# LuoGuiwen/MSM_blst

Measured on AMD Instinct MI355X. Metric: G1 MSM point-scalar pairs/sec at n=2^20, 1/2/4/8 MI355X; bit-exact vs CPU, higher is better.
Workload: dtype u32 (exact Fp381 integer arithmetic, 14x28-bit limbs)

## Files before the change

### msm_blst_amd/csrc/ches.hip

```cpp
#include <hipcub/hipcub.hpp>

#include <algorithm>
#include <cstdlib>
#include <cstring>

#include "ches_kernels.hpp"
#include "coop.hpp"
#include "engine.hpp"
#include "hoststage.hpp"
#include "pair_kernels.hpp"

#ifndef MSM_GROUP
#error "define MSM_GROUP (1 or 2)"
#endif

namespace msm {

#if MSM_GROUP == 1
static const ChesParams kChesTable[] = {
    {8, 0, 12, 22, 7, 6, 857, 10, 26},         {9, 0, 13, 20, 231, 6, 1725, 11, 24},
    {10, 0, 13, 20, 231, 6, 1725, 12, 22},     {11, 0, 14, 19, 7, 6, 3417, 13, 20},
    {12, 0, 14, 19, 7, 6, 3417, 13, 20},       {13, 0, 16, 16, 29677, 6, 18343, 15, 17},
    {14, 0, 16, 16, 29677, 6, 18343, 15, 17},  {15, 0, 16, 16, 29677, 6, 18343, 16, 16},
    {16, 0, 19, 14, 231, 6, 109244, 17, 15},   {16, 1, 18, 15, 7, 6, 54618, 17, 15},
// ... 1020 lines not shown
  const size_t fs_bytes = fg_max * n * (size_t)p_.h * 16 + 1;
  const int nfr = phase ? (int)std::max<size_t>(kFrontsMax, std::min<size_t>(kFrontPhase, ((size_t)4 << 30) / fs_bytes))
                        : nl >= 2 ? kFrontsMax : kFronts;
  const int nred = nl >= 2 ? 4 : 2;
  if ((int)fs_.size() < nfr) fs_.resize(nfr);
  for (int t = 0; t < nred; ++t) red.ensure_group(t, (int)group_max);
  const size_t sslot = n * stride;
  bool unsized = false;
  for (int f = 0; f < nfr; ++f) unsized |= fs_[f].sorted.bytes < n * (size_t)p_.h * fg_max * 4;
  static const size_t nsg_env = [] {
    const char *e = getenv("MSM_H2D_SLOTS");
    return (size_t)(e ? std::max(2, std::min(256, atoi(e))) : 0);
  }();
  const size_t slot_groups =
      std::max<size_t>(nsg_env ? nsg_env : std::max<size_t>(4, std::min<size_t>(32, ((size_t)2 << 30) / (fg_max * sslot))),
                       (size_t)nfr - 1);
  const size_t nsg = std::max<size_t>(std::min(slot_groups, nfg), (size_t)nfr - 1);
  if (scalars_on_host) scal_.ensure(slot_groups * fg_max * sslot + 16);
  if (unsized) scal_.ensure(fg_max * sslot + 16);
  for (int f = 0; f < nfr; ++f)
    if (fs_[f].sorted.bytes < n * (size_t)p_.h * fg_max * 4) {
      MSM_HIP_CHECK(hipMemsetAsync(scal_.p, 0, fg_max * sslot, s));
      digits_sort(s, scal_.as<uint8_t>(), stride, sslot, (int)fg_max, f);
      MSM_HIP_CHECK(hipStreamSynchronize(s));
    }
  const bool prof = profile_;
  profile_ = false;
  if (prof)
    while (acc_ev_.size() < std::max<size_t>(2 * count, 2 * 64)) {
      hipEvent_t e;
      MSM_HIP_CHECK(hipEventCreate(&e));
      acc_ev_.push_back(e);
    }
  while (bev_.size() < std::max<size_t>(3 * count + 2 * nfg + ngroups + 1, 3 * 64 + 3 * 64 + 1)) {
    hipEvent_t e;
    MSM_HIP_CHECK(hipEventCreateWithFlags(&e, hipEventDisableTiming));
    bev_.push_back(e);
  }
  hipEvent_t *eva = bev_.data() + 1, *evh = eva + count, *evf = evh + count, *evc = evf + nfg, *evt = evc + nfg;
  std::vector<size_t> prof_k;
  MSM_HIP_CHECK(hipEventRecord(bev_[0], s));
  MSM_HIP_CHECK(hipStreamWaitEvent(fstream_, bev_[0], 0));
  if (scalars_on_host) MSM_HIP_CHECK(hipEventSynchronize(bev_[0]));
  for (int t = 0; t < kBSets; ++t) MSM_HIP_CHECK(hipStreamWaitEvent(tails_[t], bev_[0], 0));
  auto slots = [&](size_t g) { return scal_.as<uint8_t>() + (g % nsg) * fg_max * sslot; };
  static const bool zc_env = [] {
    const char *e = getenv("MSM_ZERO_COPY_SCALARS");
    return e && atoi(e) != 0;
  }();
  bool zero_copy = false;
  if (scalars_on_host && zc_env) {
    hipPointerAttribute_t a;
    zero_copy = hipPointerGetAttributes(&a, scalars) == hipSuccess && a.type == hipMemoryTypeHost;
    if (!zero_copy) (void)hipGetLastError();
  }
  auto copy_group = [&](size_t g) {
    if (!scalars_on_host || zero_copy || g >= nfg) return;
    if (g >= nsg) MSM_HIP_CHECK(hipStreamWaitEvent(cstream_, evf[g - nsg], 0));
    for (size_t k = fgb[g]; k < fgb[g + 1]; ++k)
      MSM_HIP_CHECK(hipMemcpyAsync(slots(g) + (k - fgb[g]) * sslot, job_scalars(k), sslot, hipMemcpyHostToDevice,
                                   cstream_));
    MSM_HIP_CHECK(hipEventRecord(evc[g], cstream_));
  };
  static const bool front_after_l0 = [] {
    const char *e = getenv("MSM_FRONT_AFTER_L0");
    return e && atoi(e) != 0;
  }();
  static const size_t pace_env = [] {
    const char *e = getenv("MSM_COPY_PACE");
    return (size_t)(e ? std::max(0, std::min(32, atoi(e))) : 8);
  }();
  const size_t pace = scalars_on_host && !zero_copy && pace_env >= 3 ? pace_env : 0;
  size_t acc_enq = 0;
  auto front_group = [&](size_t g) {
    if (g >= nfg) return;
    const bool copied = scalars_on_host && !zero_copy;
    if (pace && g >= pace && g < nsg) {
      if (acc_enq) MSM_HIP_CHECK(hipEventSynchronize(eva[std::min(fgb[g] - pace, acc_enq - 1)]));
      copy_group(g);
    }
    if (copied) MSM_HIP_CHECK(hipStreamWaitEvent(fstream_, evc[g], 0));
    if (g >= (size_t)nfr) {
      const size_t last = fgb[g - nfr + 1] - 1;
      MSM_HIP_CHECK(hipStreamWaitEvent(fstream_, eva[last], 0));
      if (front_after_l0 && nl < 2) MSM_HIP_CHECK(hipStreamWaitEvent(fstream_, evh[last], 0));
      for (size_t d = 1; d < (size_t)nl && last >= d && last - d >= fgb[g - nfr]; ++d)
        MSM_HIP_CHECK(hipStreamWaitEvent(fstream_, eva[last - d], 0));
    }
    const uint8_t *src = copied ? slots(g) : job_scalars(fgb[g]);
    digits_sort(fstream_, src, stride, copied ? sslot : jstride, (int)(fgb[g + 1] - fgb[g]), (int)(g % nfr),
                fine_bt);
    MSM_HIP_CHECK(hipEventRecord(evf[g], fstream_));
  };
  for (size_t g = 0; g < (pace ? std::min(nsg, pace) : nsg); ++g) copy_group(g);
  static const int l0_env = [] {
    const char *e = getenv("MSM_ACC_AFTER_L0");
    return e ? (atoi(e) != 0 ? 1 : 0) : -1;
  }();
  const bool l0_first = l0_env < 0 ? G == 1 : l0_env == 1;
  size_t fronts_issued = 0;
  auto issue_fronts = [&](size_t upto) {
    for (; fronts_issued <= upto && fronts_issued < nfg; ++fronts_issued) front_group(fronts_issued);
  };
  const size_t nphase = phase ? std::min(nfg, (size_t)nfr) : 1;
  issue_fronts(nphase - 1);
  if (acc_groups) {
    hipStream_t lane[2] = {s, tails_[0]}, ts = tails_[1];
    for (size_t g = 0; g < nfg; ++g) {
      copy_group(g + nsg);
      const size_t k0 = fgb[g], k1 = fgb[g + 1];
      const int gb = (int)(g & 1);
      hipStream_t L = lane[gb];
      MSM_HIP_CHECK(hipStreamWaitEvent(L, evf[g], 0));
      if (g == 0 && nphase > 1) MSM_HIP_CHECK(hipStreamWaitEvent(L, evf[nphase - 1], 0));
      if (prof) MSM_HIP_CHECK(hipEventRecord(acc_ev_[2 * k0], L));
      accumulate_sets(L, (int)(g % nfr), (int)(k1 - k0), gb, job_table(k0));
      if (prof) {
        MSM_HIP_CHECK(hipEventRecord(acc_ev_[2 * k0 + 1], L));
        prof_k.push_back(k0);
      }
      for (size_t k = k0; k < k1; ++k) MSM_HIP_CHECK(hipEventRecord(eva[k], L));
      acc_enq = k1;
      for (size_t a = k0; a < k1;) {
        const size_t q = grp(a), b = std::min(k1, gfirst[q + 1]);
        if (q >= (size_t)nred) MSM_HIP_CHECK(hipStreamWaitEvent(L, evt[q - nred], 0));
        red.launch_head_slots(L, gbuckets_[gb].as<uint8_t>() + (a - k0) * NB * sizeof(Xyzz<typename FieldOf<G>::F>), NB,
                              (int)(q % nred), (int)gslot(a), (int)(b - a));
        a = b;
      }
      for (size_t k = k0; k < k1; ++k) MSM_HIP_CHECK(hipEventRecord(evh[k], L));
      for (size_t k = k0; k < k1; ++k) {
        if (!gend(k)) continue;
        const size_t q = grp(k), first = gfirst[q];
        MSM_HIP_CHECK(hipStreamWaitEvent(ts, evh[k], 0));
        if (k0 >= 1 && k0 - 1 >= first) MSM_HIP_CHECK(hipStreamWaitEvent(ts, evh[k0 - 1], 0));
        group_tail(ts, (int)(q % nred), first, k - first + 1, k + 1 == count);
        MSM_HIP_CHECK(hipEventRecord(evt[q], ts));
      }
      issue_fronts(g + nfr - 1);
    }
  }
  if (nl >= 2 && !acc_groups) {
    hipStream_t lane[3] = {s, tails_[0], tails_[1]}, ts = nl == 3 ? fstream_ : tails_[1];
    for (size_t g = 0; g < nfg; ++g) {
      copy_group(g + nsg);
      for (size_t k = fgb[g]; k < fgb[g + 1]; ++k) {
        hipStream_t L = lane[k % nl];
        const size_t q = grp(k);
        const int bset = (int)(k % nl), slot = (int)gslot(k), gset = (int)(q % nred);
        MSM_HIP_CHECK(hipStreamWaitEvent(L, evf[g], 0));
        if (q >= (size_t)nred && slot < nl)
          MSM_HIP_CHECK(hipStreamWaitEvent(L, evt[q - nred], 0));
        if (prof) MSM_HIP_CHECK(hipEventRecord(acc_ev_[2 * k], L));
        accumulate(L, (int)(g % nfr), (int)(k - fgb[g]), bset, job_table(k));
        if (prof) {
          MSM_HIP_CHECK(hipEventRecord(acc_ev_[2 * k + 1], L));
          prof_k.push_back(k);
        }
        MSM_HIP_CHECK(hipEventRecord(eva[k], L));
        acc_enq = k + 1;
        red.launch_head_slot(L, buckets_[bset].p, gset, slot);
        MSM_HIP_CHECK(hipEventRecord(evh[k], L));
        if (gend(k)) {
          for (int d = 0; d < nl && d <= slot; ++d) MSM_HIP_CHECK(hipStreamWaitEvent(ts, evh[k - d], 0));
          group_tail(ts, gset, k - slot, slot + 1, k + 1 == count);
          MSM_HIP_CHECK(hipEventRecord(evt[q], ts));
        }
      }
      issue_fronts(g + nfr - 1);
    }
  }
  static const int fuse_env = [] {
    const char *e = getenv("MSM_L0_FUSE");
    return e ? std::max(0, std::min(2, atoi(e))) : 0;
  }();
  const int fuse = nl < 2 ? fuse_env : 0;
  auto l0_group_tail = [&](size_t p) {
    const size_t pq = grp(p), pslot = gslot(p);
    if (!gend(p)) return;
    hipStream_t ts = tails_[pq % 2];
    MSM_HIP_CHECK(hipStreamWaitEvent(ts, evh[p], 0));
    group_tail(ts, (int)(pq % 2), p - pslot, pslot + 1, p + 1 == count);
    MSM_HIP_CHECK(hipEventRecord(evt[pq], ts));
  };
  auto l0_set_free = [&](size_t p) {
    const size_t pq = grp(p);
    if (gslot(p) == 0 && pq >= 2) MSM_HIP_CHECK(hipStreamWaitEvent(s, evt[pq - 2], 0));
  };
  for (size_t g = 0; g < (nl >= 2 || !fuse ? 0 : nfg); ++g) {
    copy_group(g + nsg);
    MSM_HIP_CHECK(hipStreamWaitEvent(s, evf[g], 0));
    for (size_t k = fgb[g]; k < fgb[g + 1]; ++k) {
      const int bset = (int)(k % kBSets);
      if (k >= 1) l0_set_free(k - 1);
      if (prof) MSM_HIP_CHECK(hipEventRecord(acc_ev_[2 * k], s));
      if (k >= 1)
        accumulate_l0(s, (int)(g % nfr), (int)(k - fgb[g]), bset, job_table(k), (int)((k - 1) % kBSets),
                      (int)(grp(k - 1) % 2), (int)gslot(k - 1), fuse == 2);
      else
        accumulate(s, (int)(g % nfr), (int)(k - fgb[g]), bset, job_table(k));
      if (prof) {
        MSM_HIP_CHECK(hipEventRecord(acc_ev_[2 * k + 1], s));
        prof_k.push_back(k);
      }
      MSM_HIP_CHECK(hipEventRecord(eva[k], s));
      acc_enq = k + 1;
      if (k >= 1) {
        MSM_HIP_CHECK(hipEventRecord(evh[k - 1], s));
        l0_group_tail(k - 1);
      }
    }
    issue_fronts(g + nfr - 1);
  }
  if (fuse && nl < 2) {
    const size_t p = count - 1;
    l0_set_free(p);
    red.launch_head_slot(s, buckets_[p % kBSets].p, (int)(grp(p) % 2), (int)gslot(p));
    MSM_HIP_CHECK(hipEventRecord(evh[p], s));
    l0_group_tail(p);
  }
  for (size_t g = 0; g < (nl >= 2 || fuse ? 0 : nfg); ++g) {
    copy_group(g + nsg);
    MSM_HIP_CHECK(hipStreamWaitEvent(s, evf[g], 0));
    for (size_t k = fgb[g]; k < fgb[g + 1]; ++k) {
      const int bset = (int)(k % kBSets), slot = (int)gslot(k), gset = (int)(grp(k) % 2);
      hipStream_t ts = tails_[gset];
      if (k >= (size_t)kBSets) MSM_HIP_CHECK(hipStreamWaitEvent(s, evh[k - kBSets], 0));
      if (l0_first && k >= 1) MSM_HIP_CHECK(hipStreamWaitEvent(s, evh[k - 1], 0));
      if (prof) MSM_HIP_CHECK(hipEventRecord(acc_ev_[2 * k], s));
      accumulate(s, (int)(g % nfr), (int)(k - fgb[g]), bset, job_table(k));
      if (prof) {
        MSM_HIP_CHECK(hipEventRecord(acc_ev_[2 * k + 1], s));
        prof_k.push_back(k);
      }
      MSM_HIP_CHECK(hipEventRecord(eva[k], s));
      acc_enq = k + 1;
      MSM_HIP_CHECK(hipStreamWaitEvent(ts, eva[k], 0));
      red.launch_head_slot(ts, buckets_[bset].p, gset, slot);
      MSM_HIP_CHECK(hipEventRecord(evh[k], ts));
      if (gend(k)) {
        group_tail(ts, gset, k - slot, slot + 1, k + 1 == count);
      }
    }
    issue_fronts(g + nfr - 1);
  }
  MSM_HIP_CHECK(hipEventRecord(ev_tail_[0], fstream_));
  MSM_HIP_CHECK(hipStreamWaitEvent(s, ev_tail_[0], 0));
  for (int t = 0; t < kBSets; ++t) {
    MSM_HIP_CHECK(hipEventRecord(ev_tail_[t], tails_[t]));
    MSM_HIP_CHECK(hipStreamWaitEvent(s, ev_tail_[t], 0));
  }
  for (int t = 0; t < kBSets; ++t) MSM_HIP_CHECK(hipStreamSynchronize(tails_[t]));
  MSM_HIP_CHECK(hipStreamSynchronize(fstream_));
  const size_t last_first = gfirst[ngroups - 1];
  auto combine_k = [&](size_t k) {
    outs[k] = bit_tail && k >= last_first ? red.combine_bits((const uint8_t *)host_bits_ + (k - last_first) * bb)
                                          : red.combine((const uint8_t *)host_out_ + k * ob)[0];
  };
  if (dev_out) {
  } else if (count >= 4) {
    WorkerPool::get().parallel_for(count, combine_k);
// ... 22 lines not shown
```

### msm_blst_amd/csrc/ches_kernels.hpp

```cpp
#pragma once
#include "bucket_sort.hpp"
#include "kernels.hpp"

namespace msm {

constexpr uint32_t CH_IDX_MASK = 0x00ffffffu;

__device__ constexpr uint64_t PM2[6] = {0xb9feffffffffaaa9ull, 0x1eabfffeb153ffffull, 0x6730d2a0f6b0f624ull,
                                        0x64774b84f38512bfull, 0x4b1ba7b6434bacd7ull, 0x1a0111ea397fe69aull};
__device__ __forceinline__ void fp_inv(Fp &r, const Fp &a) {
  Fp a1 = a, a2, a3, acc;
  fp_norm(a1);
  fp_sqr(a2, a1);
  fp_mul(a3, a2, a1);
  fp_one(acc);
  for (int k = 190; k >= 0; --k) {
    if (k != 190) {
      fp_sqr(acc, acc);
      fp_sqr(acc, acc);
    }
    const uint32_t w = (uint32_t)(PM2[k >> 5] >> ((k & 31) * 2)) & 3u;
    if (w) {
      const uint32_t m1 = 0u - (uint32_t)(w == 1), m2 = 0u - (uint32_t)(w == 2), m3 = 0u - (uint32_t)(w == 3);
      Fp t;
// ... 381 lines not shown
    return (int32_t)((uint32_t)((((uint64_t)hi << 32) | lo) >> sh) & qmask);
  };
  int32_t carry = 0;
  for (int j = 0; j < h - 1; ++j) carry = digit(j) + carry > qh ? 1 : 0;
  uint32_t neg = 0;
  if (digit(h - 1) + carry > qh) {
    r_minus(s);
    neg = 1u;
  }
  carry = 0;
  for (int j = 0; j < h; ++j) {
    int32_t d = digit(j) + carry;
    carry = 0;
    if (j < h - 1 && d > qh) {
      d -= q;
      carry = 1;
    }
    const size_t k = (size_t)j * n + i;
    if (d == 0) {
      keys[k] = KEY_NONE;
      continue;
    }
    uint32_t sign = (d < 0 ? 1u : 0u) ^ neg;
    uint32_t b = (uint32_t)(d < 0 ? -d : d) - 1u;
    if (j == h - 1 && b < small) {
      uint32_t c = (uint32_t)(i % copies);
      if (c) b = nb0 + (c - 1) * small + b;
    }
    keys[k] = b;
    vals[k] = (uint32_t)(i * (size_t)h + j) | (sign << 31);
  }
}

#ifndef MSM_SEGSUM_PREFETCH
#define MSM_SEGSUM_PREFETCH 0
#endif
#ifndef MSM_SEGSUM_CHAIN
#define MSM_SEGSUM_CHAIN 0
#endif
template <int G>
struct SegsumForm {
  typedef MulSplit T;
};
#if MSM_SEGSUM_CHAIN
template <>
struct SegsumForm<1> {
  typedef MulChain T;
};
#endif
template <int G>
__device__ __forceinline__ void segsum_one(const Xyzz<typename FieldOf<G>::F> *__restrict__ src,
                                           const uint32_t *__restrict__ idx, const uint32_t *__restrict__ starts,
                                           Xyzz<typename FieldOf<G>::F> *__restrict__ dst, size_t t) {
  typedef typename FieldOf<G>::F F;
  uint32_t lo = starts[t], hi = starts[t + 1];
  Xyzz<F> acc;
  if (lo == hi) {
    xyzz_set_inf(acc);
  } else {
    acc = ld16(&src[idx ? idx[lo] : lo]);
#if MSM_SEGSUM_PREFETCH
    Xyzz<F> nxt;
    if (lo + 1 < hi) nxt = ld16(&src[idx ? idx[lo + 1] : lo + 1]);
    for (uint32_t k = lo + 1; k < hi; ++k) {
      Xyzz<F> a = nxt;
      if (k + 1 < hi) nxt = ld16(&src[idx ? idx[k + 1] : k + 1]);
      xyzz_add<F, AddRegrouped<F>::value, typename SegsumForm<G>::T>(acc, a);
    }
#else
    for (uint32_t k = lo + 1; k < hi; ++k) {
      Xyzz<F> a = ld16(&src[idx ? idx[k] : k]);
      xyzz_add<F, AddRegrouped<F>::value, typename SegsumForm<G>::T>(acc, a);
    }
#endif
  }
  st16(&dst[t], acc);
}
template <int G>
static __global__ void __launch_bounds__(256)
    k_segsum(const Xyzz<typename FieldOf<G>::F> *__restrict__ src, const uint32_t *__restrict__ idx,
             const uint32_t *__restrict__ starts, Xyzz<typename FieldOf<G>::F> *__restrict__ dst, size_t nout,
             size_t src_stride, size_t dst_stride) {
  size_t t = (size_t)blockIdx.x * blockDim.x + threadIdx.x;
  if (t >= nout) return;
  segsum_one<G>(src + blockIdx.y * src_stride, idx, starts, dst + blockIdx.y * dst_stride, t);
}

template <class PT>
static __global__ void __launch_bounds__(256, MSM_ACC_WAVES)
    k_accumulate_l0(const AccSched S, const PT *__restrict__ pts, Xyzz<Fp> *__restrict__ buckets, size_t nbuckets,
                    const Xyzz<Fp> *__restrict__ l0src, const uint32_t *__restrict__ l0idx,
                    const uint32_t *__restrict__ l0starts, Xyzz<Fp> *__restrict__ l0dst, size_t l0out,
                    uint32_t l0blocks, int l0_last) {
  const uint32_t nacc = gridDim.x - l0blocks;
  const bool l0 = l0_last ? blockIdx.x >= nacc : blockIdx.x < l0blocks;
  const uint32_t b = l0 ? (l0_last ? blockIdx.x - nacc : blockIdx.x) : (l0_last ? blockIdx.x : blockIdx.x - l0blocks);
  const size_t t = (size_t)b * blockDim.x + threadIdx.x;
  if (l0) {
    if (t < l0out) segsum_one<1>(l0src, l0idx, l0starts, l0dst, t);
  } else if (t < nbuckets) {
    accumulate_bucket<1>(S, pts, buckets, t);
  }
}

template <int G>
static __global__ void __launch_bounds__(64)
    k_suffix_step(const Xyzz<typename FieldOf<G>::F> *__restrict__ in, Xyzz<typename FieldOf<G>::F> *__restrict__ out,
                  int S, int d, int W) {
  typedef typename FieldOf<G>::F F;
  size_t t = (size_t)blockIdx.x * blockDim.x + threadIdx.x;
  if (t >= (size_t)W * S) return;
  int k = (int)(t % (size_t)S);
  Xyzz<F> a = ld16(&in[t]);
  if (k + d < S) {
    Xyzz<F> b = ld16(&in[t + d]);
    xyzz_add(a, b);
  }
  st16(&out[t], a);
}
template <int G>
static __global__ void __launch_bounds__(64)
    k_pair_step(const Xyzz<typename FieldOf<G>::F> *__restrict__ in, Xyzz<typename FieldOf<G>::F> *__restrict__ out,
                size_t nout) {
  typedef typename FieldOf<G>::F F;
  size_t t = (size_t)blockIdx.x * blockDim.x + threadIdx.x;
  if (t >= nout) return;
  Xyzz<F> a = ld16(&in[2 * t]);
  Xyzz<F> b = ld16(&in[2 * t + 1]);
  xyzz_add(a, b);
  st16(&out[t], a);
}


template <int G>
__global__ void __launch_bounds__(256) k_import_xyzz(const uint64_t *__restrict__ in, Xyzz<typename FieldOf<G>::F> *__restrict__ out,
// ... 35 lines not shown
```

### include/msm_mi355x.h

```cpp
#ifndef MSM_MI355X_H
#define MSM_MI355X_H

#include <stddef.h>
#include <stdint.h>

#ifdef __cplusplus
extern "C" {
#endif

typedef uint8_t byte;
typedef uint64_t limb_t;
typedef struct { byte b[256 / 8]; } blst_scalar;
typedef struct { limb_t l[384 / 8 / sizeof(limb_t)]; } blst_fp;
typedef struct { blst_fp fp[2]; } blst_fp2;
typedef struct { blst_fp x, y, z; } blst_p1;
typedef struct { blst_fp x, y; } blst_p1_affine;
typedef struct { blst_fp2 x, y, z; } blst_p2;
typedef struct { blst_fp2 x, y; } blst_p2_affine;
typedef struct { blst_fp x, y, zzz, zz; } blst_p1xyzz;
typedef struct { blst_fp2 x, y, zzz, zz; } blst_p2xyzz;
typedef struct { int m; int b; int alpha; } digit_decomposition;

size_t blst_p1s_mult_pippenger_scratch_sizeof(size_t npoints);
void blst_p1s_mult_pippenger(blst_p1 *ret, const blst_p1_affine *const points[], size_t npoints,
// ... 68 lines not shown
                                   const int scalars[], const unsigned char booth_signs[], blst_p2xyzz buckets[],
                                   size_t q_exponent);

void blst_p1s_add(blst_p1 *ret, const blst_p1_affine *const points[], size_t npoints);
void blst_p2s_add(blst_p2 *ret, const blst_p2_affine *const points[], size_t npoints);

size_t blst_p1s_mult_wbits_precompute_sizeof(size_t wbits, size_t npoints);
void blst_p1s_mult_wbits_precompute(blst_p1_affine table[], size_t wbits, const blst_p1_affine *const points[],
                                    size_t npoints);
size_t blst_p1s_mult_wbits_scratch_sizeof(size_t npoints);
void blst_p1s_mult_wbits(blst_p1 *ret, const blst_p1_affine table[], size_t wbits, size_t npoints,
                         const byte *const scalars[], size_t nbits, limb_t *scratch);
size_t blst_p2s_mult_wbits_precompute_sizeof(size_t wbits, size_t npoints);
void blst_p2s_mult_wbits_precompute(blst_p2_affine table[], size_t wbits, const blst_p2_affine *const points[],
                                    size_t npoints);
size_t blst_p2s_mult_wbits_scratch_sizeof(size_t npoints);
void blst_p2s_mult_wbits(blst_p2 *ret, const blst_p2_affine table[], size_t wbits, size_t npoints,
                         const byte *const scalars[], size_t nbits, limb_t *scratch);

enum {
  MSM_OK = 0,
  MSM_E_ARG = -1,
  MSM_E_HIP = -2,
  MSM_E_NODEV = -3,
  MSM_E_STATE = -4
};
typedef struct msm_ctx msm_ctx;
const char *msm_last_error(void);
int msm_set_abort_on_error(int on);
int msm_error_pending(void);
int msm_device_count(void);
int msm_valu_probe(int device, double out[4]);
int msm_fp_form_ops(int device, int form, const uint32_t *in, size_t lanes, uint32_t *out);
void msm_release_engine_cache(void);
void msm_engine_cache_stats(size_t out[3]);
size_t msm_set_engine_cache_limit(size_t bytes);
int msm_register_host_table(int group, const void *rows_affine, size_t nrows);
int msm_unregister_host_table(const void *rows_affine);
int msm_ctx_create(msm_ctx **ctx, int group, int device, int window_bits);
int msm_ctx_set_points(msm_ctx *ctx, const void *points_affine, size_t npoints, int points_on_device,
                       void *hip_stream);
int msm_ctx_mult(msm_ctx *ctx, void *ret, const byte *scalars, size_t stride, size_t nbits, int scalars_on_device,
                 void *hip_stream);
int msm_ctx_mult_batch(msm_ctx *ctx, void *rets, const byte *scalars, size_t stride, size_t set_stride,
                       size_t nbits, size_t count, int scalars_on_device, void *hip_stream);
int msm_ctx_set_profiling(msm_ctx *ctx, int on);
int msm_ctx_phase_times(const msm_ctx *ctx, float out[6]);
void msm_ctx_destroy(msm_ctx *ctx);

typedef struct msm_ches_ctx msm_ches_ctx;
int msm_ches_params(int n_exp, int beta, int out[9]);
int msm_ches_ctx_create(msm_ches_ctx **ctx, int group, int device, int n_exp, int beta);
int msm_ches_ctx_create_params(msm_ches_ctx **ctx, int group, int device, const int params[9]);
int msm_ches_ctx_create_multi(msm_ches_ctx **ctx, int group, const int *devices, int ndev, int n_exp, int beta);
int msm_ches_ctx_shards(const msm_ches_ctx *ctx);
int msm_ches_ctx_rccl_exchange(const msm_ches_ctx *ctx);
int msm_ches_ctx_build_table(msm_ches_ctx *ctx, const void *points_affine, size_t npoints, int on_device,
                             void *hip_stream);
int msm_ches_ctx_set_table(msm_ches_ctx *ctx, const void *table_affine, size_t npoints, int on_device,
                           void *hip_stream);
int msm_ches_ctx_get_table(msm_ches_ctx *ctx, void *out_affine, size_t first, size_t count);
int msm_ches_ctx_mult(msm_ches_ctx *ctx, void *ret, const byte *scalars, size_t stride, int scalars_on_device,
                      void *hip_stream);
int msm_ches_ctx_mult_batch(msm_ches_ctx *ctx, void *rets, const byte *scalars, size_t stride, size_t set_stride,
                            size_t count, int scalars_on_device, void *hip_stream);
int msm_ches_ctx_save_table(msm_ches_ctx *ctx, const char *path);
// ... 135 lines not shown
```

### msm_blst_amd/csrc/abi.cpp

```cpp
#include <hip/hip_runtime.h>
#include <stdio.h>
#include <stdlib.h>
#include <string.h>

#include <algorithm>
#include <atomic>
#include <map>
#include <memory>
#include <mutex>
#include <string>

#include "../../include/msm_mi355x.h"
#include "decode.hpp"
#include "encode.hpp"
#include "engine.hpp"
#include "hash_to_curve.hpp"
#include "multi.hpp"
#include "pairing.hpp"
#include "point_segments.hpp"
#include "points_mult.hpp"
#include "pool.hpp"
#include "ptr_walk.hpp"
#include "sig_verify.hpp"
#include "table_registry.hpp"
// ... 1246 lines not shown
int msm_unregister_host_table(const void *rows) {
  if (!rows) return fail(MSM_E_ARG, "null rows");
  return TableRegistry::get().remove(rows) ? MSM_OK : fail(MSM_E_ARG, "table not registered");
}

int msm_device_count(void) {
  int n = 0;
  if (hipGetDeviceCount(&n) != hipSuccess) return 0;
  return n;
}

int msm_valu_probe(int device, double out[4]) {
  if (!out) return fail(MSM_E_ARG, "null out");
  if (msm_device_count() <= device || device < 0) return fail(MSM_E_NODEV, "no such HIP device");
  try {
    valu_probe(device, out);
    return MSM_OK;
  } catch (const std::exception &e) {
    return fail(MSM_E_HIP, e.what());
  }
}

int msm_fp_form_ops(int device, int form, const uint32_t *in, size_t lanes, uint32_t *out) {
  if (!in || !out || !lanes || (form != 0 && form != 1)) return fail(MSM_E_ARG, "bad in / out / lanes / form");
  if (msm_device_count() <= device || device < 0) return fail(MSM_E_NODEV, "no such HIP device");
  try {
    form_ops(device, form, in, lanes, out);
    return MSM_OK;
  } catch (const std::exception &e) {
    return fail(MSM_E_HIP, e.what());
  }
}

int msm_ctx_create(msm_ctx **ctx, int group, int device, int window_bits) {
  if (!ctx || (group != 1 && group != 2)) return fail(MSM_E_ARG, "bad ctx/group");
  if (msm_device_count() <= device || device < 0) return fail(MSM_E_NODEV, "no such HIP device");
  try {
    auto c = std::make_unique<msm_ctx>();
    c->group = group;
    c->device = device;
    int wb = window_bits > 0 ? window_bits : 16;
    if (group == 1) c->g1 = std::make_unique<Pippenger<1>>(device, wb);
    else c->g2 = std::make_unique<Pippenger<2>>(device, wb);
    *ctx = c.release();
    return MSM_OK;
  } catch (const std::exception &e) {
    return fail(MSM_E_HIP, e.what());
  }
}

int msm_ctx_set_points(msm_ctx *ctx, const void *points, size_t n, int on_device, void *stream) {
  if (!ctx || (!points && n)) return fail(MSM_E_ARG, "bad args");
  try {
    if (ctx->group == 1) ctx->g1->set_points(points, n, on_device != 0, (hipStream_t)stream);
    else ctx->g2->set_points(points, n, on_device != 0, (hipStream_t)stream);
    return MSM_OK;
  } catch (const std::exception &e) {
    return fail(MSM_E_HIP, e.what());
  }
}

int msm_ctx_set_points_encoded(msm_ctx *ctx, const void *src, size_t n, int encoding, int flags, int src_on_device,
                               size_t *first_bad, void *stream) {
  if (!ctx || (!src && n)) return fail(MSM_E_ARG, "bad args");
  if (n == 0) return msm_ctx_set_points(ctx, nullptr, 0, 1, stream);
  std::vector<uint8_t> st;
// ... 640 lines not shown
```

### msm_blst_amd/csrc/ec.hpp

```cpp
#pragma once
#include "fp.hpp"

namespace msm {

template <class F>
struct Aff {
  F x, y;
};
template <class F>
struct Xyzz {
  F x, y, zzz, zz;
};

template <class F>
MSM_FN bool xyzz_is_inf(const Xyzz<F> &a) {
  return f_is_zero_exact(a.zz);
}
template <class F>
MSM_FN void xyzz_set_inf(Xyzz<F> &a) {
  f_zero(a.x);
  f_zero(a.y);
  f_zero(a.zzz);
  f_zero(a.zz);
}
// ... 5 lines not shown
    f_nred(r.y);
  } else {
    r.y = p.y;
  }
  f_one(r.zzz);
  f_one(r.zz);
}

template <class F, class CF = MulSplit>
MSM_FN void xyzz_dbl(Xyzz<F> &r, const Xyzz<F> &a) {
  if (xyzz_is_inf(a)) {
    r = a;
    return;
  }
  F U, V, W, S, M, t, X3;
  f_add(U, a.y, a.y);
  f_sqr(V, U, CF{});
  f_mul(W, V, U, CF{});
  f_mul(S, a.x, V, CF{});
  f_mul(r.zz, V, a.zz, CF{});
  f_mul(r.zzz, W, a.zzz, CF{});
  f_sqr(M, a.x, CF{});
  f_mul3(M, M);
  f_sqr(X3, M, CF{});
  F z;
  f_zero(z);
  f_sub_2x(X3, X3, z, S);
  f_norm(X3);
  f_sub16(t, S, X3);
  f_mul_sub(r.y, t, M, W, a.y, CF{});
  r.x = X3;
}

template <class F, class CF = MulSplit>
MSM_FN void xyzz_madd(Xyzz<F> &acc, const Aff<F> &p, bool neg, bool acc_affine = false) {
  if (xyzz_is_inf(acc)) {
    xyzz_from_aff(acc, p, neg);
    return;
  }
  F y2, P, R, PP, PPP, t;
  if (neg) {
    f_neg4(y2, p.y);
  } else {
    y2 = p.y;
  }
  if (acc_affine) {
    P = p.x;
    if (neg) f_nred(y2);
    R = y2;
  } else {
    f_mul_bs(P, p.x, acc.zz, CF{});
    f_mul_bs(R, y2, acc.zzz, CF{});
  }
  f_sub16(P, P, acc.x);
  f_sub4(R, R, acc.y);
  f_sqr(PP, P, CF{});
  if (__builtin_expect(f_is_zero_S(PP), 0)) {
    F RR;
    f_sqr(RR, R, CF{});
    if (f_is_zero_S(RR)) {
      Xyzz<F> b = acc;
      xyzz_dbl<F, CF>(acc, b);
    } else {
      xyzz_set_inf(acc);
    }
    return;
  }
  if (!__builtin_constant_p(acc_affine)) f_pin(PP);
  if (acc_affine) {
    acc.zz = PP;
  } else {
    f_mul_bs(acc.zz, acc.zz, PP, CF{});
  }
  f_mul_bs(PPP, P, PP, CF{});
  f_mul_bs(acc.x, acc.x, PP, CF{});
  if (acc_affine) {
    acc.zzz = PPP;
  } else {
    f_mul_bs(acc.zzz, acc.zzz, PPP, CF{});
  }
  F X3;
  f_sqr(X3, R, CF{});
  f_sub_2x(X3, X3, PPP, acc.x);
  f_norm(X3);
  f_sub16(t, acc.x, X3);
  f_mul_sub(acc.y, t, R, acc.y, PPP, CF{});
  acc.x = X3;
}

template <class F, class CF = MulSplit>
MSM_FN void xyzz_add_u1s1(Xyzz<F> &acc, const Xyzz<F> &b) {
  F P, R, PP, PPP, t;
  f_mul_bs(acc.x, acc.x, b.zz, CF{});
  f_mul_bs(acc.y, acc.y, b.zzz, CF{});
  f_mul_bs(P, b.x, acc.zz, CF{});
  f_sub4(P, P, acc.x);
  f_mul_bs(R, b.y, acc.zzz, CF{});
  f_sub4(R, R, acc.y);
  f_mul_bs(acc.zz, acc.zz, b.zz, CF{});
  f_mul_bs(acc.zzz, acc.zzz, b.zzz, CF{});
  f_sqr(PP, P, CF{});
  if (__builtin_expect(f_is_zero_S(PP), 0)) {
    F RR;
    f_sqr(RR, R, CF{});
    if (f_is_zero_S(RR)) {
      Xyzz<F> a = acc;
      xyzz_dbl<F, CF>(acc, a);
    } else {
      xyzz_set_inf(acc);
    }
    return;
  }
  f_mul_bs(acc.zz, acc.zz, PP, CF{});
  f_mul_bs(PPP, P, PP, CF{});
  f_mul_bs(acc.x, acc.x, PP, CF{});
  f_mul_bs(acc.zzz, acc.zzz, PPP, CF{});
  F X3;
  f_sqr(X3, R, CF{});
  f_sub_2x(X3, X3, PPP, acc.x);
  f_norm(X3);
// ... 59 lines not shown
```

### msm_blst_amd/csrc/engine.hpp

```cpp
#pragma once
#include <hip/hip_runtime.h>
#include <stdint.h>

#include <cstdlib>
#include <memory>
#include <stdexcept>
#include <string>
#include <vector>

#include "acc_sched.hpp"
#include "host_fp.hpp"

#define MSM_HIP_CHECK(x)                                                                           \
  do {                                                                                            \
    hipError_t e_ = (x);                                                                          \
    if (e_ != hipSuccess)                                                                         \
      throw std::runtime_error(std::string("HIP error ") + hipGetErrorString(e_) + " at " + #x); \
  } while (0)

namespace msm {

class HostStager;

inline unsigned nblk(size_t n, unsigned b) { return (unsigned)((n + b - 1) / b); }
// ... 370 lines not shown
class Wbits {
 public:
  typedef typename HostField<G>::F HF;
  Wbits(int device, int wbits);
  void precompute(const void *points_blst, size_t n, bool on_device, hipStream_t s);
  void set_table(const void *table_blst, size_t n, bool on_device, hipStream_t s);
  void get_table(void *out_blst, size_t first, size_t count, hipStream_t s);
  void run(hipStream_t s, const uint8_t *d_scalars, size_t stride, int nbits, hfp::Jac<HF> *out);
  void upload_scalars(const void *host, size_t bytes, hipStream_t s);
  size_t npoints() const { return n_; }
  size_t table_rows() const { return n_ << (wbits_ - 1); }
  int wbits() const { return wbits_; }
  int device() const { return dev_; }
  size_t device_bytes() const { return table_.bytes + parts_[0].bytes + parts_[1].bytes + fin_.bytes + scal_.bytes; }

 private:
  int dev_, wbits_;
  size_t n_ = 0;
  DevBuf table_, parts_[2], fin_, scal_;
};

template <int G>
void entry_msm(void *ret_jac, const void *pts_blst, size_t npts, const uint32_t *keys, const uint32_t *vals,
               size_t ne, size_t nb, const uint32_t *weights, void *buckets_out);
typedef void (*EntryFill)(void *ctx, size_t t0, size_t t1, uint32_t *keys, uint32_t *vals);
template <int G>
void entry_msm_ptrs(void *ret, const void *const *points, size_t ne, EntryFill fill, void *fill_ctx, size_t nb,
                    const uint32_t *weights, void *buckets_out);
template <int G>
void weighted_bucket_sum(void *ret_jac, const void *buckets_blst, size_t nb, const uint32_t *weights);

void valu_probe(int device, double out[4]);
void form_ops(int device, int form, const uint32_t *in, size_t lanes, uint32_t *out);
template <int G>
void test_field(int op, const uint64_t *a, const uint64_t *b, uint64_t *out, size_t n);
template <int G>
void test_xyzz(const uint64_t *pts, size_t npts, const uint32_t *ops, int len, size_t nseq, uint64_t *out);

struct DeviceGuard {
  int prev = -1;
  explicit DeviceGuard(int dev) {
    MSM_HIP_CHECK(hipGetDevice(&prev));
    if (prev != dev) MSM_HIP_CHECK(hipSetDevice(dev));
  }
  ~DeviceGuard() {
    int cur = -1;
    if (hipGetDevice(&cur) == hipSuccess && cur != prev && prev >= 0) (void)hipSetDevice(prev);
  }
};

}
```

### msm_blst_amd/csrc/probe.hip

```cpp
#include <hip/hip_runtime.h>

#include <algorithm>
#include <cstring>

#include "kernels.hpp"
#include "engine.hpp"

namespace msm {
namespace {

__global__ void __launch_bounds__(256) k_probe_mad(uint64_t *out, uint32_t seed, int iters) {
  const uint32_t t = threadIdx.x + blockIdx.x * blockDim.x;
  uint64_t acc[16];
  const uint32_t a = t | 1, b = seed | 3;
#pragma unroll
  for (int k = 0; k < 16; ++k) acc[k] = t + k;
  for (int it = 0; it < iters; ++it) {
#pragma unroll
    for (int k = 0; k < 16; ++k)
      asm volatile("v_mad_u64_u32 %0, vcc, %1, %2, %0" : "+v"(acc[k]) : "v"(a), "v"(b) : "vcc");
  }
  uint64_t s = 0;
#pragma unroll
  for (int k = 0; k < 16; ++k) s += acc[k];
// ... 30 lines not shown
  for (int it = 0; it < 2 * iters; ++it) {
    const Aff<Fp> p = pts[it & 3];
    xyzz_madd(acc, p, (it & 2) != 0);
  }
  uint32_t s = 0;
#pragma unroll
  for (int i = 0; i < NL; ++i) s ^= acc.x.v[i] ^ acc.y.v[i] ^ acc.zzz.v[i] ^ acc.zz.v[i];
  out[t] = s;
}

template <class CF>
__global__ void __launch_bounds__(256) k_form_ops(const Fp *__restrict__ in, Fp *__restrict__ out, size_t lanes) {
  const size_t t = (size_t)blockIdx.x * blockDim.x + threadIdx.x;
  if (t >= lanes) return;
  const Fp *a = in + t * 8;
  Fp *o = out + t * 11;
  Fp r;
  fp_mul(r, a[0], a[1], CF{});
  o[0] = r;
  fp_sqr(r, a[0], CF{});
  o[1] = r;
  fp_mul2(r, a[0], a[1], a[2], a[3], CF{});
  o[2] = r;
  Xyzz<Fp> q = {a[0], a[1], a[2], a[3]};
  const Aff<Fp> p = {a[4], a[5]};
  xyzz_madd<Fp, CF>(q, p, (t & 1) != 0);
  o[3] = q.x, o[4] = q.y, o[5] = q.zzz, o[6] = q.zz;
  q = {a[0], a[1], a[2], a[3]};
  const Xyzz<Fp> b = {a[4], a[5], a[6], a[7]};
  xyzz_add<Fp, true, CF>(q, b);
  o[7] = q.x, o[8] = q.y, o[9] = q.zzz, o[10] = q.zz;
}

template <class L>
float best_ms(L launch) {
  hipEvent_t e0, e1;
  MSM_HIP_CHECK(hipEventCreate(&e0));
  MSM_HIP_CHECK(hipEventCreate(&e1));
  launch();
  MSM_HIP_CHECK(hipGetLastError());
  MSM_HIP_CHECK(hipDeviceSynchronize());
  float best = 1e30f;
  for (int r = 0; r < 3; ++r) {
    MSM_HIP_CHECK(hipEventRecord(e0, 0));
    launch();
    MSM_HIP_CHECK(hipEventRecord(e1, 0));
    MSM_HIP_CHECK(hipEventSynchronize(e1));
    float ms = 0;
    MSM_HIP_CHECK(hipEventElapsedTime(&ms, e0, e1));
    best = std::min(best, ms);
  }
  (void)hipEventDestroy(e0);
  (void)hipEventDestroy(e1);
  return best;
}

}

void valu_probe(int device, double out[4]) {
  {
    DeviceGuard g(device);
    int cus = 0;
    MSM_HIP_CHECK(hipDeviceGetAttribute(&cus, hipDeviceAttributeMultiprocessorCount, device));
    DevBuf obuf, pbuf;
    obuf.ensure((size_t)cus * 8 * 256 * 8);
    Aff<Fp> h[4];
// ... 24 lines not shown
      total += 4 * ms;
      fpm = std::max(fpm, (double)blocks * 256 * iters * 2 / (ms * 1e-3));
    }
    for (int bpc : {3, 6}) {
      const int blocks = cus * bpc, iters = 64;
      const float ms = best_ms([&] {
        hipLaunchKernelGGL(k_probe_madd, dim3(blocks), dim3(256), 0, 0, obuf.as<uint32_t>(), pbuf.as<Aff<Fp>>(),
                           iters);
      });
      total += 4 * ms;
      madd = std::max(madd, (double)blocks * 256 * iters * 2 / (ms * 1e-3));
    }
    out[0] = mad;
    out[1] = fpm;
    out[2] = madd;
    out[3] = total;
  }
}

void form_ops(int device, int form, const uint32_t *in, size_t lanes, uint32_t *out) {
  DeviceGuard g(device);
  DevBuf ibuf, obuf;
  ibuf.ensure(lanes * 8 * sizeof(Fp));
  obuf.ensure(lanes * 11 * sizeof(Fp));
  MSM_HIP_CHECK(hipMemcpy(ibuf.p, in, lanes * 8 * sizeof(Fp), hipMemcpyHostToDevice));
  const dim3 grid((unsigned)((lanes + 255) / 256));
  if (form) hipLaunchKernelGGL(k_form_ops<MulChain>, grid, dim3(256), 0, 0, ibuf.as<Fp>(), obuf.as<Fp>(), lanes);
  else hipLaunchKernelGGL(k_form_ops<MulSplit>, grid, dim3(256), 0, 0, ibuf.as<Fp>(), obuf.as<Fp>(), lanes);
  MSM_HIP_CHECK(hipGetLastError());
  MSM_HIP_CHECK(hipDeviceSynchronize());
  MSM_HIP_CHECK(hipMemcpy(out, obuf.p, lanes * 11 * sizeof(Fp), hipMemcpyDeviceToHost));
}

}
```

Baseline: 483.9 million.

## Add kernel-based H2D scalar staging and pace host copies on accumulate start

Adds an opt-in path, MSM_H2D_STAGE, that copies host scalars into the device slot buffers with a vectorized non-temporal-load GPU kernel reading mapped host memory, in place of per-job hipMemcpyAsync. That path can run on the copy or front stream and is gated on stream events with a configurable lead. The default pacing of host scalar copies also changes. When fewer than two accumulation lanes are used, the host now waits on new per-job accumulate-start events with a shorter pace, not on accumulate-end events, so copies can be issued earlier. This adds event bookkeeping, and earlier copies may contend with accumulation for PCIe and memory bandwidth.

```diff
diff --git a/msm_blst_amd/csrc/ches.hip b/msm_blst_amd/csrc/ches.hip
--- a/msm_blst_amd/csrc/ches.hip
+++ b/msm_blst_amd/csrc/ches.hip
@@ -1076,22 +1076,53 @@
       MSM_HIP_CHECK(hipEventCreate(&e));
       acc_ev_.push_back(e);
     }
-  while (bev_.size() < std::max<size_t>(3 * count + 2 * nfg + ngroups + 1, 3 * 64 + 3 * 64 + 1)) {
+  while (bev_.size() < std::max<size_t>(4 * count + 2 * nfg + ngroups + 1, 4 * 64 + 3 * 64 + 1)) {
     hipEvent_t e;
     MSM_HIP_CHECK(hipEventCreateWithFlags(&e, hipEventDisableTiming));
     bev_.push_back(e);
   }
-  hipEvent_t *eva = bev_.data() + 1, *evh = eva + count, *evf = evh + count, *evc = evf + nfg, *evt = evc + nfg;
+  hipEvent_t *eva = bev_.data() + 1, *evh = eva + count, *evf = evh + count, *evc = evf + nfg, *evt = evc + nfg,
+             *evs = evt + ngroups;
   std::vector<size_t> prof_k;
   MSM_HIP_CHECK(hipEventRecord(bev_[0], s));
   MSM_HIP_CHECK(hipStreamWaitEvent(fstream_, bev_[0], 0));
-  if (scalars_on_host) MSM_HIP_CHECK(hipEventSynchronize(bev_[0]));
   for (int t = 0; t < kBSets; ++t) MSM_HIP_CHECK(hipStreamWaitEvent(tails_[t], bev_[0], 0));
   auto slots = [&](size_t g) { return scal_.as<uint8_t>() + (g % nsg) * fg_max * sslot; };
   static const bool zc_env = [] {
     const char *e = getenv("MSM_ZERO_COPY_SCALARS");
     return e && atoi(e) != 0;
   }();
+  static const int stage_env = [] {
+    const char *e = getenv("MSM_H2D_STAGE");
+    return e ? std::max(0, std::min(2, atoi(e))) : 0;
+  }();
+  static const size_t stage_lead = [] {
+    const char *e = getenv("MSM_STAGE_LEAD");
+    return (size_t)(e ? std::max(2, std::min(32, atoi(e))) : 3);
+  }();
+  static const unsigned stage_wgs = [] {
+    const char *e = getenv("MSM_STAGE_WGS");
+    return (unsigned)(e ? std::max(1, std::min(1024, atoi(e))) : 32);
+  }();
+  const uint8_t *mapped = nullptr;
+  int stage = 0;
+  if (scalars_on_host && stage_env && !zc_env && ((uintptr_t)scalars | set_stride | sslot) % 16 == 0) {
+    const size_t span = (nsets - 1) * set_stride + nseg * sslot;
+    void *d0 = nullptr, *d1 = nullptr;
+    if (hipHostGetDevicePointer(&d0, const_cast<uint8_t *>(scalars), 0) == hipSuccess &&
+        hipHostGetDevicePointer(&d1, const_cast<uint8_t *>(scalars) + span - 1, 0) == hipSuccess &&
+        static_cast<uint8_t *>(d1) - static_cast<uint8_t *>(d0) == (ptrdiff_t)(span - 1)) {
+      mapped = static_cast<const uint8_t *>(d0);
+      stage = stage_env;
+    } else {
+      (void)hipGetLastError();
+    }
+  }
+  hipStream_t hs = stage == 2 ? fstream_ : cstream_;
+  if (stage == 1)
+    MSM_HIP_CHECK(hipStreamWaitEvent(cstream_, bev_[0], 0));
+  else if (scalars_on_host && !stage)
+    MSM_HIP_CHECK(hipEventSynchronize(bev_[0]));
   bool zero_copy = false;
   if (scalars_on_host && zc_env) {
     hipPointerAttribute_t a;
@@ -1100,27 +1131,52 @@
   }
   auto copy_group = [&](size_t g) {
     if (!scalars_on_host || zero_copy || g >= nfg) return;
-    if (g >= nsg) MSM_HIP_CHECK(hipStreamWaitEvent(cstream_, evf[g - nsg], 0));
-    for (size_t k = fgb[g]; k < fgb[g + 1]; ++k)
-      MSM_HIP_CHECK(hipMemcpyAsync(slots(g) + (k - fgb[g]) * sslot, job_scalars(k), sslot, hipMemcpyHostToDevice,
-                                   cstream_));
-    MSM_HIP_CHECK(hipEventRecord(evc[g], cstream_));
+    if (g >= nsg) MSM_HIP_CHECK(hipStreamWaitEvent(hs, evf[g - nsg], 0));
+    if (stage) {
+      k_stage_scalars<<<dim3(stage_wgs, (unsigned)(fgb[g + 1] - fgb[g])), 256, 0, hs>>>(
+          mapped + (job_scalars(fgb[g]) - scalars), jstride, slots(g), sslot, sslot);
+      MSM_HIP_CHECK(hipGetLastError());
+    } else {
+      for (size_t k = fgb[g]; k < fgb[g + 1]; ++k)
+        MSM_HIP_CHECK(hipMemcpyAsync(slots(g) + (k - fgb[g]) * sslot, job_scalars(k), sslot, hipMemcpyHostToDevice,
+                                     cstream_));
+    }
+    MSM_HIP_CHECK(hipEventRecord(evc[g], hs));
   };
   static const bool front_after_l0 = [] {
     const char *e = getenv("MSM_FRONT_AFTER_L0");
     return e && atoi(e) != 0;
   }();
-  static const size_t pace_env = [] {
+  static const int at_start_env = [] {
+    const char *e = getenv("MSM_COPY_AT_START");
+    return e ? (atoi(e) != 0 ? 1 : 0) : -1;
+  }();
+  static const int pace_env = [] {
     const char *e = getenv("MSM_COPY_PACE");
-    return (size_t)(e ? std::max(0, std::min(32, atoi(e))) : 8);
-  }();
-  const size_t pace = scalars_on_host && !zero_copy && pace_env >= 3 ? pace_env : 0;
+    return e ? std::max(0, std::min(32, atoi(e))) : -1;
+  }();
+  const bool want_start = at_start_env < 0 ? nl < 2 : at_start_env == 1;
+  const size_t pace_val = pace_env >= 0 ? (size_t)pace_env : want_start ? 5 : 8;
+  const size_t pace = scalars_on_host && !zero_copy && !stage && pace_val >= 3 ? pace_val : 0;
+  const bool at_start = pace && want_start;
+  const bool mark = stage == 1 || at_start;
+  auto mark_start = [&](size_t k, hipStream_t L) {
+    if (mark) MSM_HIP_CHECK(hipEventRecord(evs[k], L));
+  };
   size_t acc_enq = 0;
   auto front_group = [&](size_t g) {
     if (g >= nfg) return;
     const bool copied = scalars_on_host && !zero_copy;
     if (pace && g >= pace && g < nsg) {
-      if (acc_enq) MSM_HIP_CHECK(hipEventSynchronize(eva[std::min(fgb[g] - pace, acc_enq - 1)]));
+      if (acc_enq && at_start)
+        MSM_HIP_CHECK(hipEventSynchronize(evs[std::min(fgb[g] - (pace - 1), acc_enq - 1)]));
+      else if (acc_enq)
+        MSM_HIP_CHECK(hipEventSynchronize(eva[std::min(fgb[g] - pace, acc_enq - 1)]));
+      copy_group(g);
+    }
+    if (stage && g < nsg) {
+      if (stage == 1 && acc_enq && fgb[g] >= stage_lead)
+        MSM_HIP_CHECK(hipStreamWaitEvent(cstream_, evs[std::min(fgb[g] - stage_lead, acc_enq - 1)], 0));
       copy_group(g);
     }
     if (copied) MSM_HIP_CHECK(hipStreamWaitEvent(fstream_, evc[g], 0));
@@ -1136,7 +1192,7 @@
                 fine_bt);
     MSM_HIP_CHECK(hipEventRecord(evf[g], fstream_));
   };
-  for (size_t g = 0; g < (pace ? std::min(nsg, pace) : nsg); ++g) copy_group(g);
+  for (size_t g = 0; g < (stage ? 0 : pace ? std::min(nsg, pace) : nsg); ++g) copy_group(g);
   static const int l0_env = [] {
     const char *e = getenv("MSM_ACC_AFTER_L0");
     return e ? (atoi(e) != 0 ? 1 : 0) : -1;
@@ -1157,6 +1213,7 @@
       hipStream_t L = lane[gb];
       MSM_HIP_CHECK(hipStreamWaitEvent(L, evf[g], 0));
       if (g == 0 && nphase > 1) MSM_HIP_CHECK(hipStreamWaitEvent(L, evf[nphase - 1], 0));
+      for (size_t k = k0; k < k1; ++k) mark_start(k, L);
       if (prof) MSM_HIP_CHECK(hipEventRecord(acc_ev_[2 * k0], L));
       accumulate_sets(L, (int)(g % nfr), (int)(k1 - k0), gb, job_table(k0));
       if (prof) {
@@ -1195,6 +1252,7 @@
         MSM_HIP_CHECK(hipStreamWaitEvent(L, evf[g], 0));
         if (q >= (size_t)nred && slot < nl)
           MSM_HIP_CHECK(hipStreamWaitEvent(L, evt[q - nred], 0));
+        mark_start(k, L);
         if (prof) MSM_HIP_CHECK(hipEventRecord(acc_ev_[2 * k], L));
         accumulate(L, (int)(g % nfr), (int)(k - fgb[g]), bset, job_table(k));
         if (prof) {
@@ -1237,6 +1295,7 @@
     for (size_t k = fgb[g]; k < fgb[g + 1]; ++k) {
       const int bset = (int)(k % kBSets);
       if (k >= 1) l0_set_free(k - 1);
+      mark_start(k, s);
       if (prof) MSM_HIP_CHECK(hipEventRecord(acc_ev_[2 * k], s));
       if (k >= 1)
         accumulate_l0(s, (int)(g % nfr), (int)(k - fgb[g]), bset, job_table(k), (int)((k - 1) % kBSets),
@@ -1271,6 +1330,7 @@
       hipStream_t ts = tails_[gset];
       if (k >= (size_t)kBSets) MSM_HIP_CHECK(hipStreamWaitEvent(s, evh[k - kBSets], 0));
       if (l0_first && k >= 1) MSM_HIP_CHECK(hipStreamWaitEvent(s, evh[k - 1], 0));
+      mark_start(k, s);
       if (prof) MSM_HIP_CHECK(hipEventRecord(acc_ev_[2 * k], s));
       accumulate(s, (int)(g % nfr), (int)(k - fgb[g]), bset, job_table(k));
       if (prof) {
diff --git a/msm_blst_amd/csrc/ches_kernels.hpp b/msm_blst_amd/csrc/ches_kernels.hpp
--- a/msm_blst_amd/csrc/ches_kernels.hpp
+++ b/msm_blst_amd/csrc/ches_kernels.hpp
@@ -437,6 +437,25 @@
   }
 }
 
+typedef uint32_t stage_v4 __attribute__((ext_vector_type(4)));
+static __global__ void __launch_bounds__(256)
+    k_stage_scalars(const uint8_t *__restrict__ src, size_t src_stride, uint8_t *__restrict__ dst, size_t dst_stride,
+                    size_t bytes) {
+  const stage_v4 *sv = reinterpret_cast<const stage_v4 *>(src + blockIdx.y * src_stride);
+  stage_v4 *dv = reinterpret_cast<stage_v4 *>(dst + blockIdx.y * dst_stride);
+  const size_t nv = bytes / 16, T = (size_t)gridDim.x * blockDim.x;
+  size_t i = (size_t)blockIdx.x * blockDim.x + threadIdx.x;
+  for (; i + 3 * T < nv; i += 4 * T) {
+    const stage_v4 a = __builtin_nontemporal_load(sv + i), b = __builtin_nontemporal_load(sv + i + T),
+                   c = __builtin_nontemporal_load(sv + i + 2 * T), d = __builtin_nontemporal_load(sv + i + 3 * T);
+    dv[i] = a;
+    dv[i + T] = b;
+    dv[i + 2 * T] = c;
+    dv[i + 3 * T] = d;
+  }
+  for (; i < nv; i += T) dv[i] = __builtin_nontemporal_load(sv + i);
+}
+
 #ifndef MSM_SEGSUM_PREFETCH
 #define MSM_SEGSUM_PREFETCH 0
 #endif
```

New measurement: 477.5 million. 0.987x the previous value.

## Unify bucket accumulation and L0 segment-sum into one generalized madd loop

Applied to the files above, without the earlier changes.

Rewrites the fused accumulate/L0 kernel so both block roles run a single loop calling a generalized XYZZ mixed-add. That add optionally treats the second operand as full XYZZ by scaling with its zz/zzz. The aim is to remove divergent code paths and code-size/register pressure from inlining two different routines into one kernel. The L0 path now pays extra field multiplications per add, and the shared loop adds branches on the role flag. A probe kernel and ABI entry are added to test the generalized add.

```diff
diff --git a/include/msm_mi355x.h b/include/msm_mi355x.h
--- a/include/msm_mi355x.h
+++ b/include/msm_mi355x.h
@@ -124,6 +124,7 @@
 int msm_device_count(void);
 int msm_valu_probe(int device, double out[4]);
 int msm_fp_form_ops(int device, int form, const uint32_t *in, size_t lanes, uint32_t *out);
+int msm_fp_madd_general_ops(int device, const uint32_t *in, size_t lanes, uint32_t *out);
 void msm_release_engine_cache(void);
 void msm_engine_cache_stats(size_t out[3]);
 size_t msm_set_engine_cache_limit(size_t bytes);
diff --git a/msm_blst_amd/csrc/abi.cpp b/msm_blst_amd/csrc/abi.cpp
--- a/msm_blst_amd/csrc/abi.cpp
+++ b/msm_blst_amd/csrc/abi.cpp
@@ -1302,6 +1302,17 @@
   }
 }
 
+int msm_fp_madd_general_ops(int device, const uint32_t *in, size_t lanes, uint32_t *out) {
+  if (!in || !out || !lanes) return fail(MSM_E_ARG, "bad in / out / lanes");
+  if (msm_device_count() <= device || device < 0) return fail(MSM_E_NODEV, "no such HIP device");
+  try {
+    madd_general_ops(device, in, lanes, out);
+    return MSM_OK;
+  } catch (const std::exception &e) {
+    return fail(MSM_E_HIP, e.what());
+  }
+}
+
 int msm_ctx_create(msm_ctx **ctx, int group, int device, int window_bits) {
   if (!ctx || (group != 1 && group != 2)) return fail(MSM_E_ARG, "bad ctx/group");
   if (msm_device_count() <= device || device < 0) return fail(MSM_E_NODEV, "no such HIP device");
diff --git a/msm_blst_amd/csrc/ches_kernels.hpp b/msm_blst_amd/csrc/ches_kernels.hpp
--- a/msm_blst_amd/csrc/ches_kernels.hpp
+++ b/msm_blst_amd/csrc/ches_kernels.hpp
@@ -497,15 +497,44 @@
                     const Xyzz<Fp> *__restrict__ l0src, const uint32_t *__restrict__ l0idx,
                     const uint32_t *__restrict__ l0starts, Xyzz<Fp> *__restrict__ l0dst, size_t l0out,
                     uint32_t l0blocks, int l0_last) {
+  typedef typename AccForm<1>::T CF;
   const uint32_t nacc = gridDim.x - l0blocks;
   const bool l0 = l0_last ? blockIdx.x >= nacc : blockIdx.x < l0blocks;
   const uint32_t b = l0 ? (l0_last ? blockIdx.x - nacc : blockIdx.x) : (l0_last ? blockIdx.x : blockIdx.x - l0blocks);
   const size_t t = (size_t)b * blockDim.x + threadIdx.x;
+  if (t >= (l0 ? l0out : nbuckets)) return;
+  const uint32_t *ip = l0idx;
+  uint32_t istr = 1, k = 0, end;
   if (l0) {
-    if (t < l0out) segsum_one<1>(l0src, l0idx, l0starts, l0dst, t);
-  } else if (t < nbuckets) {
-    accumulate_bucket<1>(S, pts, buckets, t);
-  }
+    k = l0starts[t], end = l0starts[t + 1];
+  } else {
+    const PayloadStream ps(S, (uint32_t)t);
+    ip = ps.p, istr = ps.stride, end = S.counts[t];
+  }
+  const uint8_t *base = l0 ? reinterpret_cast<const uint8_t *>(l0src) : reinterpret_cast<const uint8_t *>(pts);
+  const uint32_t esz = l0 ? (uint32_t)sizeof(Xyzz<Fp>) : (uint32_t)sizeof(PT);
+  auto element = [&](uint32_t j) {
+    const uint32_t e = ip ? ip[(size_t)j * istr] : j;
+    return e;
+  };
+  Xyzz<Fp> acc;
+  xyzz_set_inf(acc);
+  if (l0 && k < end) {
+    acc = ld16(reinterpret_cast<const Xyzz<Fp> *>(base + (size_t)element(k) * esz));
+    ++k;
+  }
+  bool fresh = false;
+  for (; k < end; ++k) {
+    const uint32_t e = element(k);
+    const uint8_t *row = base + (size_t)(e & 0x7fffffffu) * esz;
+    const Aff<Fp> p = ld16(reinterpret_cast<const Aff<Fp> *>(row));
+    if (f_is_zero_exact(p.x) && f_is_zero_exact(p.y)) continue;
+    const bool start = !l0 && xyzz_is_inf(acc);
+    xyzz_madd_general<Fp, CF, false>(acc, p, reinterpret_cast<const Xyzz<Fp> *>(row), !l0 && (e >> 31) != 0, fresh,
+                                     l0);
+    fresh = start;
+  }
+  st16(l0 ? &l0dst[t] : &buckets[S.order[t]], acc);
 }
 
 template <int G>
diff --git a/msm_blst_amd/csrc/ec.hpp b/msm_blst_amd/csrc/ec.hpp
--- a/msm_blst_amd/csrc/ec.hpp
+++ b/msm_blst_amd/csrc/ec.hpp
@@ -61,25 +61,47 @@
   r.x = X3;
 }
 
-template <class F, class CF = MulSplit>
-MSM_FN void xyzz_madd(Xyzz<F> &acc, const Aff<F> &p, bool neg, bool acc_affine = false) {
+template <class T>
+MSM_FN const T *ptr_again(const T *p) {
+#ifndef MSM_FP_HOST_TEST
+  asm volatile("" : "+v"(p));
+#endif
+  return p;
+}
+template <class F, class CF>
+MSM_FN void xyzz_madd_core(Xyzz<F> &acc, const F &x2, const F &y2in, const Xyzz<F> *b2, bool neg, bool acc_affine,
+                           bool general) {
   if (xyzz_is_inf(acc)) {
-    xyzz_from_aff(acc, p, neg);
-    return;
-  }
+    if (general) {
+      acc.x = x2, acc.y = y2in, acc.zzz = b2->zzz, acc.zz = b2->zz;
+    } else {
+      const Aff<F> p = {x2, y2in};
+      xyzz_from_aff(acc, p, neg);
+    }
+    return;
+  }
+  if (general) f_mul_bs(acc.x, acc.x, b2->zz, CF{});
   F y2, P, R, PP, PPP, t;
   if (neg) {
-    f_neg4(y2, p.y);
-  } else {
-    y2 = p.y;
+    f_neg4(y2, y2in);
+  } else {
+    y2 = y2in;
   }
   if (acc_affine) {
-    P = p.x;
+    P = x2;
     if (neg) f_nred(y2);
     R = y2;
   } else {
-    f_mul_bs(P, p.x, acc.zz, CF{});
+    f_mul_bs(P, x2, acc.zz, CF{});
     f_mul_bs(R, y2, acc.zzz, CF{});
+  }
+  if (general) {
+    const Xyzz<F> *b = ptr_again(b2);
+    const F zz2 = b->zz;
+    f_mul_bs(acc.zz, acc.zz, zz2, CF{});
+    const F zzz2 = b->zzz;
+    f_mul_bs(acc.y, acc.y, zzz2, CF{});
+    f_mul_bs(acc.zzz, acc.zzz, zzz2, CF{});
   }
   f_sub16(P, P, acc.x);
   f_sub4(R, R, acc.y);
@@ -115,6 +137,16 @@
   f_sub16(t, acc.x, X3);
   f_mul_sub(acc.y, t, R, acc.y, PPP, CF{});
   acc.x = X3;
+}
+template <class F, class CF = MulSplit>
+MSM_FN void xyzz_madd(Xyzz<F> &acc, const Aff<F> &p, bool neg, bool acc_affine = false) {
+  xyzz_madd_core<F, CF>(acc, p.x, p.y, nullptr, neg, acc_affine, false);
+}
+template <class F, class CF = MulSplit, bool TEST_INF = true>
+MSM_FN void xyzz_madd_general(Xyzz<F> &acc, const Aff<F> &xy, const Xyzz<F> *b, bool neg, bool acc_affine,
+                              bool general) {
+  if (TEST_INF && general && f_is_zero_exact(b->zz)) return;
+  xyzz_madd_core<F, CF>(acc, xy.x, xy.y, b, neg && !general, acc_affine && !general, general);
 }
 
 template <class F, class CF = MulSplit>
diff --git a/msm_blst_amd/csrc/engine.hpp b/msm_blst_amd/csrc/engine.hpp
--- a/msm_blst_amd/csrc/engine.hpp
+++ b/msm_blst_amd/csrc/engine.hpp
@@ -426,6 +426,7 @@
 
 void valu_probe(int device, double out[4]);
 void form_ops(int device, int form, const uint32_t *in, size_t lanes, uint32_t *out);
+void madd_general_ops(int device, const uint32_t *in, size_t lanes, uint32_t *out);
 template <int G>
 void test_field(int op, const uint64_t *a, const uint64_t *b, uint64_t *out, size_t n);
 template <int G>
diff --git a/msm_blst_amd/csrc/probe.hip b/msm_blst_amd/csrc/probe.hip
--- a/msm_blst_amd/csrc/probe.hip
+++ b/msm_blst_amd/csrc/probe.hip
@@ -86,6 +86,23 @@
   o[7] = q.x, o[8] = q.y, o[9] = q.zzz, o[10] = q.zz;
 }
 
+__global__ void __launch_bounds__(256) k_madd_general_ops(const Fp *__restrict__ in, Fp *__restrict__ out,
+                                                          size_t lanes) {
+  const size_t t = (size_t)blockIdx.x * blockDim.x + threadIdx.x;
+  if (t >= lanes) return;
+  const Fp *a = in + t * 8;
+  Fp *o = out + t * 8;
+  const Xyzz<Fp> *b = reinterpret_cast<const Xyzz<Fp> *>(a + 4);
+  Xyzz<Fp> q = {a[0], a[1], a[2], a[3]};
+  const Aff<Fp> xy = {a[4], a[5]};
+  if (!(f_is_zero_exact(xy.x) && f_is_zero_exact(xy.y))) xyzz_madd_general<Fp, MulChain, false>(q, xy, b, false, false, true);
+  o[0] = q.x, o[1] = q.y, o[2] = q.zzz, o[3] = q.zz;
+  q = {a[0], a[1], a[2], a[3]};
+  const Xyzz<Fp> bb = {a[4], a[5], a[6], a[7]};
+  xyzz_add<Fp, true, MulSplit>(q, bb);
+  o[4] = q.x, o[5] = q.y, o[6] = q.zzz, o[7] = q.zz;
+}
+
 template <class L>
 float best_ms(L launch) {
   hipEvent_t e0, e1;
@@ -176,4 +193,17 @@
   MSM_HIP_CHECK(hipMemcpy(out, obuf.p, lanes * 11 * sizeof(Fp), hipMemcpyDeviceToHost));
 }
 
-}
+void madd_general_ops(int device, const uint32_t *in, size_t lanes, uint32_t *out) {
+  DeviceGuard g(device);
+  DevBuf ibuf, obuf;
+  ibuf.ensure(lanes * 8 * sizeof(Fp));
+  obuf.ensure(lanes * 8 * sizeof(Fp));
+  MSM_HIP_CHECK(hipMemcpy(ibuf.p, in, lanes * 8 * sizeof(Fp), hipMemcpyHostToDevice));
+  hipLaunchKernelGGL(k_madd_general_ops, dim3((unsigned)((lanes + 255) / 256)), dim3(256), 0, 0, ibuf.as<Fp>(),
+                     obuf.as<Fp>(), lanes);
+  MSM_HIP_CHECK(hipGetLastError());
+  MSM_HIP_CHECK(hipDeviceSynchronize());
+  MSM_HIP_CHECK(hipMemcpy(out, obuf.p, lanes * 8 * sizeof(Fp), hipMemcpyDeviceToHost));
+}
+
+}
```

After: 455.7 million before, 454.0 million after. No clear change (-0.4%).
